# ilur98/DLMC-QUANT

Hardware: AMD Instinct MI355X
Metric: ResNet-50 W8A8 fake-quant fwd images/sec (higher is better)
Workload: dtype i8; 1 GPU; resnet50 W8A8 per-channel fake-quant forward (FSPTQ forms: W minmax_channel s8, A minmax_tensor u8), BN folded first as in FSPTQuant.py:67, fused int8 MFMA conv/linear, frozen execution plan (epilogue-fused ReLU / shortcut / next-layer codes; block end + next 1x1 as one launch; weight codes quantised once at plan build), 2 HIP streams per GPU, 224x224 relu(N(0,1)) pixels, batch 512 per GPU, scales; global_batch=512, parallelism=dp1 (batch-sharded replicas)

## Files before the change

### dlmc-quant_amd/csrc/conv3x3_i8.hip

```cpp
#include "conv_i8_common.h"

namespace dlmcq {

struct HaloGeom {
  int N, H, W, C, K;
  int Hin, Win;
  int Wp, FS;
  uint32_t MQ;
  int nblk_n;
  int hp;
  FastDiv fsdiv, wpdiv;
};

constexpr int halo_tap(bool s2, int t) { return !s2 ? t : (t == 0 ? 4 : t == 1 ? 3 : t == 2 ? 5 : t == 3 ? 1 : t == 4 ? 7 : t == 5 ? 0 : t == 6 ? 2 : t == 7 ? 6 : 8); }
constexpr int halo_ph(bool s2, int t) { return !s2 ? 0 : (t == 0 ? 0 : t <= 2 ? 1 : t <= 4 ? 2 : 3); }
constexpr int halo_rs(bool s2, int t) { return !s2 ? t / 3 : (halo_tap(true, t) / 3 > 0 ? 1 : 0); }
constexpr int halo_cs(bool s2, int t) { return !s2 ? t % 3 : (halo_tap(true, t) % 3 > 0 ? 1 : 0); }

template <int BN, int TM, int NW, int WC, int HPW, int NHB, int WPE, bool XS, int LAB = 0, bool S2 = false, int HPA = HPW * NW, bool PLAIN = false>
__global__ __launch_bounds__(NW * 64, WPE) void conv3x3_halo_i8_kernel(
    const int8_t* __restrict__ x, const int8_t* __restrict__ w, const float* __restrict__ bias, const int32_t* __restrict__ wsum,
    const float* __restrict__ s_in, const float* __restrict__ zp_in, const float* __restrict__ s_w, HaloGeom g, int shift, ConvEpi ep,
    unsigned long long* __restrict__ trace) {
  constexpr bool STAMP = LAB == 1;
  if (LAB >= 9 && LAB <= 11 && blockIdx.x >= 256 && blockIdx.x < 512) {
    for (int i = 0; i < (LAB == 9 ? 4 : LAB == 10 ? 2 : 8); ++i) __builtin_amdgcn_s_sleep(127);
  }
  if ((LAB == 12 || LAB == 13) && blockIdx.x < 1024) {
    for (int i = 0; i < (int)((blockIdx.x >> 8) & 3u); ++i) {
      if (LAB == 12) __builtin_amdgcn_s_sleep(127);
      else __builtin_amdgcn_s_sleep(63);
    }
  }
  const unsigned long long t_start = STAMP ? __builtin_readcyclecounter() : 0ull;
  constexpr int NT = NW * 64;
  constexpr int NBUF = 3;
  constexpr int SLAB = BN * 64;
  constexpr int WPX = NW / WC;
  constexpr int PW = TM / WPX;
  constexpr int CW = BN / WC;
  constexpr int PB = PW / 32, CB = CW / 32;
  constexpr int HP = HPA;
  constexpr int HALO = HP * 1024;
  constexpr int NBW = SLAB / 1024 / NW;
  constexpr int RING = NBUF * SLAB;
  constexpr int SROW = BN + 16;
  constexpr int STAGE = TM * SROW;
  constexpr int OPER = RING + NHB * HALO;
  constexpr int LDS_BYTES = OPER < STAGE ? STAGE : OPER;
  constexpr int PAR_BYTES = 3 * BN * 4;
  static_assert(PB >= 1 && CB >= 1 && NBW >= 1 && NBW * NW * 1024 == SLAB && HPW <= 8 && BN % 64 == 0 && (S2 ? NHB == 3 : (NHB == 1 || NHB == 2)) && HPA <= HPW * NW, "tile shape");
  __shared__ __attribute__((aligned(1024))) int8_t lds[LDS_BYTES + PAR_BYTES];
  int8_t* const ring = lds;
  int8_t* const halo = lds + RING;
  int8_t* const par = lds + LDS_BYTES;
  const uint32_t nwg = gridDim.x;
  const uint32_t xcd = blockIdx.x & 7u, slot = blockIdx.x >> 3;
  const uint32_t qd = nwg >> 3, rm = nwg & 7u;
  const uint32_t tile = (xcd < rm ? xcd * (qd + 1) : rm * (qd + 1) + (xcd - rm) * qd) + slot;
  const int bn = tile % g.nblk_n, bm = tile / g.nblk_n;
  const uint32_t q0 = (uint32_t)bm * TM;
  const int n0 = bn * BN;

  const int tid = threadIdx.x, wave = __builtin_amdgcn_readfirstlane(tid >> 6), lane = tid & 63, l31 = lane & 31, hsel = lane >> 5;
  const int wc = wave % WC, wp = wave / WC;
  unsigned long long* const wgt = (STAMP && tid == 0) ? trace + 64 * 8 + 6 * (size_t)blockIdx.x : nullptr;
  unsigned long long* const stp = (STAMP && tid == 0 && blockIdx.x == gridDim.x / 2) ? trace : nullptr;
  if (STAMP && wgt) {
    wgt[0] = t_start;
    wgt[4] = __builtin_amdgcn_s_memrealtime();
  }
  int stepno = 0;
  auto stamp = [&](int k) {
    if (STAMP && stp && stepno < 64) stp[stepno * 8 + k] = __builtin_readcyclecounter();
  };

  {
    const void* arrs[3] = {s_w, wsum, bias};
#pragma unroll
    for (int a = 0; a < 3; ++a) {
      if (!arrs[a]) continue;
#pragma unroll
      for (int c = 0; c < BN / 64; ++c) {
        if (((a * (BN / 64) + c) % NW) != wave) continue;
        __builtin_amdgcn_global_load_lds((gptr_t)(static_cast<const int32_t*>(arrs[a]) + n0 + c * 64 + lane),
                                         (lptr_t)(par + (a * BN + c * 64) * 4), 4, 0, 0);
      }
    }
  }
  const float zpf = zp_in ? zp_in[0] : 0.0f;
  const int zpi = (int)__builtin_rintf(zpf);
  const float sin_early = s_in[0];
  const uint32_t xorw = 0x80808080u;
  const int8_t* const padline = g_pad_table.b + ((zpi & 0xff) << 6);

  const int lrow = lane >> 2, pslot = lane & 3;
  const int8_t* hsrc[HPW];
  int hinc[HPW];
  int hpc[HPW];
#pragma unroll
  for (int i = 0; i < HPW; ++i) {
    int pc = i * NW + wave;
    pc = pc < g.hp ? pc : g.hp - 1;
    hpc[i] = pc;
    const int p = pc * 16 + lrow;
    const uint32_t f = q0 + (uint32_t)p;
    const uint32_t n = fdiv(f, g.fsdiv);
    const uint32_t rem = f - n * (uint32_t)g.FS;
    const uint32_t fy = fdiv(rem, g.wpdiv);
    const uint32_t fx = rem - fy * (uint32_t)g.Wp;
    const bool in = n < (uint32_t)g.N && fy >= 1u && fx >= 1u;
    const int seg = pslot ^ ((p >> 2) & 3);
    if constexpr (S2) {
      hsrc[i] = in ? x + ((int64_t)((n * (uint32_t)g.Hin + 2u * (fy - 1u)) * (uint32_t)g.Win + 2u * (fx - 1u))) * g.C + seg * 16 : padline;
      hinc[i] = in ? -1 : 0;
    } else {
      hsrc[i] = in ? x + ((int64_t)((n * (uint32_t)g.H + fy - 1u) * (uint32_t)g.W + fx - 1u)) * g.C + seg * 16 : padline;
      hinc[i] = in ? 64 : 0;
    }
  }
  auto issue_halo = [&](auto i_c, int buf) {
    constexpr int i = decltype(i_c)::value;
    if (LAB != 3) __builtin_amdgcn_global_load_lds((gptr_t)hsrc[i], (lptr_t)(halo + buf * HALO + hpc[i] * 1024), 16, 0, 0);
    hsrc[i] += hinc[i];
  };
  const int ph_row = g.Win * g.C, ph_col = g.C;
  auto issue_tile = [&](int ph, int c, int buf) {
    const int off = (ph >> 1) * ph_row + (ph & 1) * ph_col + c * 64;
    static_for<HPW>([&](auto i_c) {
      constexpr int i = decltype(i_c)::value;
      if (LAB != 3) __builtin_amdgcn_global_load_lds((gptr_t)(hsrc[i] + (off & hinc[i])), (lptr_t)(halo + buf * HALO + hpc[i] * 1024), 16, 0, 0);
    });
  };

  const int8_t* wsrc[NBW];
#pragma unroll
  for (int j = 0; j < NBW; ++j) {
    const int drow = (j * NW + wave) * 16 + lrow, d = drow & 31;
    const int k = n0 + (drow & ~31) + 16 * ((d >> 2) & 1) + 4 * (d >> 3) + (d & 3);
    wsrc[j] = w + (int64_t)k * (9 * g.C) + halo_tap(S2, 0) * g.C + (pslot ^ ((drow >> 2) & 3)) * 16;
  }
  const int nchunks = g.C >> 6;
  auto issue_w = [&](auto slot_c, auto u_c) {
    constexpr int SL = decltype(slot_c)::value, u = decltype(u_c)::value;
    constexpr int dtap = u == 8 ? halo_tap(S2, 0) - halo_tap(S2, 8) : halo_tap(S2, (u + 1) % 9) - halo_tap(S2, u);
    const int inc = dtap * g.C + (u == 8 ? 64 : 0);
#pragma unroll
    for (int j = 0; j < NBW; ++j) {
      if (LAB != 2) __builtin_amdgcn_global_load_lds((gptr_t)wsrc[j], (lptr_t)(ring + SL * SLAB + (j * NW + wave) * 1024), 16, 0, 0);
      wsrc[j] += inc;
    }
  };

  int woff[2];
  {
    const int d = wc * CW + l31;
    woff[0] = d * 64 + ((hsel ^ ((d >> 2) & 3)) << 4);
    woff[1] = woff[0] ^ 32;
  }
  const int pbase = wp * PW + l31;
  const int tap_r1 = g.Wp, tap_r2 = 2 * g.Wp;

  i32x16 acc[CB][PB];
#pragma unroll
  for (int jc = 0; jc < CB; ++jc)
#pragma unroll
    for (int jp = 0; jp < PB; ++jp)
#pragma unroll
      for (int i = 0; i < 16; ++i) acc[jc][jp][i] = 0;

  i32x4 wfA[CB], pfA[PB], wfB[CB], pfB[PB];
  auto read_frags = [&](auto u_c, auto t_c, auto ks_c, const int8_t* hbuf, i32x4 (&wf)[CB], i32x4 (&pf)[PB]) {
    constexpr int U = decltype(u_c)::value, t = decltype(t_c)::value, ks = decltype(ks_c)::value;
    const int p0 = pbase + (halo_rs(S2, t) == 0 ? 0 : (halo_rs(S2, t) == 1 ? tap_r1 : tap_r2)) + halo_cs(S2, t);
    const int pa = (p0 * 64 + ((hsel ^ ((p0 >> 2) & 3)) << 4)) ^ (ks << 5);
    const int8_t* const sb = ring + U * SLAB;
#pragma unroll
    for (int jc = 0; jc < CB; ++jc) wf[jc] = *reinterpret_cast<const i32x4*>(sb + woff[ks] + jc * 2048);
#pragma unroll
    for (int jp = 0; jp < PB; ++jp) pf[jp] = *reinterpret_cast<const i32x4*>(hbuf + pa + jp * 2048);
  };
  auto multiply = [&](const i32x4 (&wf)[CB], i32x4 (&pf)[PB]) {
    if (XS && LAB != 6) {
#pragma unroll
      for (int jp = 0; jp < PB; ++jp)
        pf[jp] = i32x4{(int)(pf[jp].x ^ xorw), (int)(pf[jp].y ^ xorw), (int)(pf[jp].z ^ xorw), (int)(pf[jp].w ^ xorw)};
    }
#pragma unroll
    for (int jc = 0; jc < CB; ++jc)
#pragma unroll
      for (int jp = 0; jp < PB; ++jp) {
        if (LAB == 4) asm volatile("" ::"v"(wf[jc]), "v"(pf[jp]));
        else acc[jc][jp] = __builtin_amdgcn_mfma_i32_32x32x32_i8(wf[jc], pf[jp], acc[jc][jp], 0, 0, 0);
      }
  };
  constexpr int nbw = (LAB == 2 ? 0 : NBW);

  if constexpr (S2) {
    issue_tile(0, 0, 0);
    issue_tile(1, 0, 1);
    issue_tile(2, 0, 2);
  } else {
    static_for<HPW>([&](auto i) { issue_halo(i, 0); });
  }
  issue_w(std::integral_constant<int, 0>{}, std::integral_constant<int, 0>{});
  issue_w(std::integral_constant<int, 1>{}, std::integral_constant<int, 1>{});
  issue_w(std::integral_constant<int, 2>{}, std::integral_constant<int, 2>{});
  if (STAMP && wgt) wgt[1] = __builtin_readcyclecounter();
  asm volatile("s_waitcnt vmcnt(%0)\n\ts_barrier" ::"n"(2 * nbw) : "memory");
  if (tid < BN) {
    float* pf = reinterpret_cast<float*>(par) + tid;
    int* pi = reinterpret_cast<int*>(par) + BN + tid;
    *pf = sin_early * *pf;
    *pi = (shift - zpi) * *pi;
  }
  read_frags(std::integral_constant<int, 0>{}, std::integral_constant<int, 0>{}, std::integral_constant<int, 0>{}, halo, wfA, pfA);

  for (int c = 0; c < (NHB == 1 ? 1 : nchunks); ++c) {
    const bool more = NHB != 1 && c + 1 < nchunks;
    const int b0 = S2 ? c % 3 : (NHB == 2 ? (c & 1) : 0);
    auto tile_of = [&](int ph, bool next_chunk) -> const int8_t* {
      if constexpr (S2) {
        int b = b0 + ph + (next_chunk ? 1 : 0);
        b = b >= 6 ? b - 6 : (b >= 3 ? b - 3 : b);
        return halo + b * HALO;
      } else {
        return halo + (NHB == 2 ? ((next_chunk ? c + 1 : c) & 1) * HALO : 0);
      }
    };
    static_for<9>([&](auto t_c) {
      constexpr int t = decltype(t_c)::value;
      constexpr int U = t % NBUF;
      stamp(0);
      read_frags(std::integral_constant<int, U>{}, t_c, std::integral_constant<int, 1>{}, tile_of(halo_ph(S2, t), false), wfB, pfB);
      multiply(wfA, pfA);
      stamp(1);
      if (t < 8 || more) {
        constexpr int hw = (LAB == 3 ? 0 : (S2 ? HPW : 1));
        if constexpr (S2) {
          if (t >= 7 && !more) asm volatile("s_waitcnt vmcnt(0) lgkmcnt(0)\n\ts_barrier" ::: "memory");
          else if (t == 1 || (t == 0 && c > 0) || ((t == 3 || t == 5) && more))
            asm volatile("s_waitcnt vmcnt(%0) lgkmcnt(0)\n\ts_barrier" ::"n"(nbw + hw) : "memory");
          else asm volatile("s_waitcnt vmcnt(%0) lgkmcnt(0)\n\ts_barrier" ::"n"(nbw) : "memory");
        } else {
          constexpr bool HPREV = t >= 1 && t <= HPW && t <= 7;
          if (t >= 7 && !more) asm volatile("s_waitcnt vmcnt(0) lgkmcnt(0)\n\ts_barrier" ::: "memory");
          else if (HPREV && more) asm volatile("s_waitcnt vmcnt(%0) lgkmcnt(0)\n\ts_barrier" ::"n"(nbw + hw) : "memory");
          else asm volatile("s_waitcnt vmcnt(%0) lgkmcnt(0)\n\ts_barrier" ::"n"(nbw) : "memory");
        }
        stamp(2);
        read_frags(std::integral_constant<int, (U + 1) % NBUF>{}, std::integral_constant<int, (t + 1) % 9>{}, std::integral_constant<int, 0>{},
                   tile_of(halo_ph(S2, (t + 1) % 9), t == 8), wfA, pfA);
        if constexpr (S2) {
          if constexpr (t == 0) issue_tile(3, c, b0);
          if constexpr (t == 2 || t == 4 || t == 8) {
            if (more) issue_tile(t == 2 ? 0 : (t == 4 ? 1 : 2), c + 1, (b0 + (t == 2 ? 1 : (t == 4 ? 2 : 0))) % 3);
          }
        } else if constexpr (t < HPW && NHB == 2) {
          if (more) issue_halo(t_c, (c + 1) & 1);
        }
        if (t < 6 || more) issue_w(std::integral_constant<int, U>{}, std::integral_constant<int, (t + 3) % 9>{});
        stamp(3);
      }
      multiply(wfB, pfB);
      if (STAMP) {
        asm volatile("s_nop 0" ::"v"(acc[0][0][0]), "v"(acc[CB - 1][PB - 1][15]));
        stamp(4);
        ++stepno;
      }
    });
  }
  if (STAMP && wgt) wgt[2] = __builtin_readcyclecounter();

  asm volatile("s_barrier" ::: "memory");
  const EpiQuant eq(ep, ep.relu != 0);
  int8_t* const stg = lds;
  auto row_addr = [&](int rr, bool& ok) -> uint8_t* {
    const uint32_t q = q0 + (uint32_t)rr;
    const uint32_t n = fdiv(q, g.fsdiv);
    const uint32_t rem = q - n * (uint32_t)g.FS;
    const uint32_t yy = fdiv(rem, g.wpdiv);
    const uint32_t xx = rem - yy * (uint32_t)g.Wp;
    ok = q < g.MQ && yy < (uint32_t)g.H && xx < (uint32_t)g.W;
    return ep.codes + ((int64_t)((n * (uint32_t)g.H + yy) * (uint32_t)g.W + xx)) * g.K + n0;
  };
#pragma unroll
  for (int jp = 0; jp < PB; ++jp) {
    bool ok8 = false;
    uint8_t* dst8 = nullptr;
    if (LAB == 8) dst8 = row_addr(wp * PW + jp * 32 + l31, ok8);
#pragma unroll
    for (int jc = 0; jc < CB; ++jc) {
      const int cb = wc * CW + jc * 32 + hsel * 16;
      f32x4 y[4];
#pragma unroll
      for (int q = 0; q < 4; ++q) {
        const f32x4 mu = *reinterpret_cast<const f32x4*>(par + (cb + 4 * q) * 4);
        const i32x4 co = *reinterpret_cast<const i32x4*>(par + (BN + cb + 4 * q) * 4);
        const f32x4 bs = bias ? *reinterpret_cast<const f32x4*>(par + (2 * BN + cb + 4 * q) * 4) : f32x4{0.0f, 0.0f, 0.0f, 0.0f};
        if constexpr (PLAIN) {
          const f32x2 ya = pk_fma(f32x2{(float)(acc[jc][jp][4 * q] + co.x), (float)(acc[jc][jp][4 * q + 1] + co.y)}, f32x2{mu.x, mu.y}, f32x2{bs.x, bs.y});
          const f32x2 yb = pk_fma(f32x2{(float)(acc[jc][jp][4 * q + 2] + co.z), (float)(acc[jc][jp][4 * q + 3] + co.w)}, f32x2{mu.z, mu.w}, f32x2{bs.z, bs.w});
          y[q] = f32x4{ya.x, ya.y, yb.x, yb.y};
        } else {
          y[q] = f32x4{dequant1(acc[jc][jp][4 * q] + co.x, mu.x, bs.x), dequant1(acc[jc][jp][4 * q + 1] + co.y, mu.y, bs.y),
                       dequant1(acc[jc][jp][4 * q + 2] + co.z, mu.z, bs.z), dequant1(acc[jc][jp][4 * q + 3] + co.w, mu.w, bs.w)};
        }
      }
      uint32_t wq[4];
      bool uq[4];
      if (LAB == 7) {
#pragma unroll
        for (int q = 0; q < 4; ++q) wq[q] = __builtin_bit_cast(uint32_t, y[q].x + y[q].y + y[q].z + y[q].w);
      } else if constexpr (PLAIN) eq.code4n_plain(y, wq);
      else eq.code4n(y, wq, uq);
      const i32x4 c16 = i32x4{(int)wq[0], (int)wq[1], (int)wq[2], (int)wq[3]};
      if (LAB == 8) {
        if (ok8) __builtin_nontemporal_store(c16, reinterpret_cast<i32x4*>(dst8 + cb));
      } else *reinterpret_cast<i32x4*>(stg + (wp * PW + jp * 32 + l31) * SROW + cb) = c16;
    }
  }
  if (LAB != 8) {
    constexpr int LPR = BN / 16;
    if constexpr (WC == 1) {
      asm volatile("s_waitcnt lgkmcnt(0)" ::: "memory");
      constexpr int RPP = 64 / LPR;
      const int srow = lane / LPR, sseg = lane % LPR;
#pragma unroll
      for (int it = 0; it < PW / RPP; ++it) {
        const int rr = wp * PW + it * RPP + srow;
        bool ok;
        uint8_t* const dst = row_addr(rr, ok);
        const i32x4 c16 = *reinterpret_cast<const i32x4*>(stg + rr * SROW + sseg * 16);
        if (ok) __builtin_nontemporal_store(c16, reinterpret_cast<i32x4*>(dst + sseg * 16));
      }
    } else {
      __syncthreads();
      constexpr int RPP = NT / LPR;
      const int srow = tid / LPR, sseg = tid % LPR;
#pragma unroll
      for (int it = 0; it < TM / RPP; ++it) {
        const int rr = it * RPP + srow;
        bool ok;
        uint8_t* const dst = row_addr(rr, ok);
        const i32x4 c16 = *reinterpret_cast<const i32x4*>(stg + rr * SROW + sseg * 16);
        if (ok) __builtin_nontemporal_store(c16, reinterpret_cast<i32x4*>(dst + sseg * 16));
      }
    }
  }
  if (STAMP && wgt) {
    asm volatile("s_waitcnt vmcnt(0)" ::: "memory");
    wgt[3] = __builtin_readcyclecounter();
    wgt[5] = __builtin_amdgcn_s_memrealtime();
  }
}

bool conv3x3_halo_applies(int64_t N, int64_t H, int64_t W, int64_t C, int64_t K, int64_t R, int64_t S, int32_t stride, int32_t pad,
                          int32_t dilation, const ConvEpi& ep, const float* out, bool dual) {
  if (R != 3 || S != 3 || (stride != 1 && stride != 2) || pad != 1 || dilation != 1 || dual || out || ep.residual || ep.w_off || !ep.codes)
    return false;
  if (C % 64 != 0 || K % 64 != 0 || !aligned16(ep.codes)) return false;
  if (ep.relu == DLMCQ_ACT_RELU6) return false;
  if (stride == 2 && ((H | W) & 1)) return false;
  const int64_t P = H / stride, Q = W / stride;
  if (stride == 2 && Q + 1 > 62) return false;
  if (stride == 2 && C == 64 && K != 64) return false;
  if (Q + 1 > 120 || N * (P + 1) * (Q + 1) + 1024 >= (1ll << 31) || N * H * W * C >= (1ll << 31)) return false;
  return true;
}

int conv3x3_halo_launch(const int8_t* x, const int8_t* w, const float* bias, const int32_t* wsum, const float* in_scale,
                        const float* in_zero_point, const float* w_scale, int64_t N, int64_t H, int64_t W, int64_t C, int64_t K,
                        int32_t stride, int shift, const ConvEpi& ep, hipStream_t st, int lab, void* lab_trace) {
  constexpr int TM = 256;
  const int bn = K % 128 == 0 ? 128 : 64;
  const bool s2 = stride == 2;
  const bool plain = epi_plain(ep);
  HaloGeom g;
  g.N = (int)N; g.Hin = (int)H; g.Win = (int)W; g.H = (int)(H / stride); g.W = (int)(W / stride); g.C = (int)C; g.K = (int)K;
  g.Wp = g.W + 1;
  g.FS = (g.H + 1) * (g.W + 1);
  g.MQ = (uint32_t)(N * g.FS);
  g.nblk_n = (int)(K / bn);
  g.hp = (TM + (s2 ? 1 : 2) * g.Wp + 2 + 15) / 16;
  g.fsdiv = make_fastdiv((uint32_t)g.FS);
  g.wpdiv = make_fastdiv((uint32_t)g.Wp);
  const int64_t nblk_m = ((int64_t)g.MQ + TM - 1) / TM;
  const int64_t nwg = nblk_m * g.nblk_n;
  if (nwg >= (1ll << 31)) return DLMCQ_ERANGE;
  unsigned long long* const trace = static_cast<unsigned long long*>(lab_trace);
#define DLMCQ_HALO_ARGS(NW) dim3((uint32_t)nwg), dim3(NW * 64), 0, st, x, w, bias, wsum, in_scale, in_zero_point, w_scale, g, shift, ep, trace
#ifdef DLMCQ_LAB
  if (lab) {
    const int v = lab % 100;
    if (s2 || g.hp > 24 || (v == 1 && !trace)) return DLMCQ_EINVAL;
    if (lab >= 100) {
      if (bn != 128) return DLMCQ_EINVAL;
      switch (v) {
#define DLMCQ_HALO_LAB(V) case V: hipLaunchKernelGGL((conv3x3_halo_i8_kernel<128, TM, 8, 2, 3, 2, 4, true, V>), DLMCQ_HALO_ARGS(8)); break
        DLMCQ_HALO_LAB(0); DLMCQ_HALO_LAB(1); DLMCQ_HALO_LAB(4);
#undef DLMCQ_HALO_LAB
        default: return DLMCQ_EINVAL;
      }
    } else if (bn == 128) {
      switch (v) {
#define DLMCQ_HALO_LAB(V) case V: hipLaunchKernelGGL((conv3x3_halo_i8_kernel<128, TM, 4, 1, 6, 2, 2, true, V>), DLMCQ_HALO_ARGS(4)); break
        DLMCQ_HALO_LAB(1); DLMCQ_HALO_LAB(2); DLMCQ_HALO_LAB(3); DLMCQ_HALO_LAB(4); DLMCQ_HALO_LAB(6); DLMCQ_HALO_LAB(7); DLMCQ_HALO_LAB(8);
        DLMCQ_HALO_LAB(9); DLMCQ_HALO_LAB(10); DLMCQ_HALO_LAB(11);
#undef DLMCQ_HALO_LAB
        default: return DLMCQ_EINVAL;
      }
    } else {
      if (C != 64) return DLMCQ_EINVAL;
      switch (v) {
#define DLMCQ_HALO_LAB(V) case V: hipLaunchKernelGGL((conv3x3_halo_i8_kernel<64, TM, 4, 1, 6, 1, 4, true, V>), DLMCQ_HALO_ARGS(4)); break
        DLMCQ_HALO_LAB(1); DLMCQ_HALO_LAB(2); DLMCQ_HALO_LAB(3); DLMCQ_HALO_LAB(4); DLMCQ_HALO_LAB(6); DLMCQ_HALO_LAB(7); DLMCQ_HALO_LAB(8);
        DLMCQ_HALO_LAB(12); DLMCQ_HALO_LAB(13);
#undef DLMCQ_HALO_LAB
        default: return DLMCQ_EINVAL;
      }
    }
    return launch_status();
  }
#else
  if (lab) return DLMCQ_EINVAL;
#endif
#define DLMCQ_HALO_GO(NW, ...)                                                                            \
  do {                                                                                                   \
    if (shift) hipLaunchKernelGGL((conv3x3_halo_i8_kernel<__VA_ARGS__>), DLMCQ_HALO_ARGS(NW));           \
    else hipLaunchKernelGGL((conv3x3_halo_i8_kernel<__VA_ARGS__>), DLMCQ_HALO_ARGS(NW));                 \
  } while (0)
  if (s2) {
    if (g.hp > 20) return DLMCQ_EINVAL;
    const bool big = g.hp > 18;
#define DLMCQ_HALO_S2(BN_, HPA_, WPE_)                                                                                                         \
  do {                                                                                                                                        \
    if (shift && plain) hipLaunchKernelGGL((conv3x3_halo_i8_kernel<BN_, TM, 4, 1, 5, 3, WPE_, true, 0, true, HPA_, true>), DLMCQ_HALO_ARGS(4));  \
    else if (shift) hipLaunchKernelGGL((conv3x3_halo_i8_kernel<BN_, TM, 4, 1, 5, 3, WPE_, true, 0, true, HPA_>), DLMCQ_HALO_ARGS(4));            \
    else if (plain) hipLaunchKernelGGL((conv3x3_halo_i8_kernel<BN_, TM, 4, 1, 5, 3, WPE_, false, 0, true, HPA_, true>), DLMCQ_HALO_ARGS(4));     \
    else hipLaunchKernelGGL((conv3x3_halo_i8_kernel<BN_, TM, 4, 1, 5, 3, WPE_, false, 0, true, HPA_>), DLMCQ_HALO_ARGS(4));                      \
  } while (0)
    if (bn == 128) {
      if (!big) DLMCQ_HALO_S2(128, 18, 2);
      else DLMCQ_HALO_S2(128, 20, 1);
    } else {
      if (!big) DLMCQ_HALO_S2(64, 18, 2);
      else DLMCQ_HALO_S2(64, 20, 2);
    }
#undef DLMCQ_HALO_S2
    return launch_status();
  }
  if (g.hp > 32) return DLMCQ_EINVAL;
  const bool wide = g.hp > 24;
#undef DLMCQ_HALO_GO
#define DLMCQ_HALO_GO(BN_, HPW_, NHB_, WPE_)                                                                                                              \
  do {                                                                                                                                                   \
    if (shift && plain) hipLaunchKernelGGL((conv3x3_halo_i8_kernel<BN_, TM, 4, 1, HPW_, NHB_, WPE_, true, 0, false, 4 * HPW_, true>), DLMCQ_HALO_ARGS(4));  \
    else if (shift) hipLaunchKernelGGL((conv3x3_halo_i8_kernel<BN_, TM, 4, 1, HPW_, NHB_, WPE_, true>), DLMCQ_HALO_ARGS(4));                                \
    else if (plain) hipLaunchKernelGGL((conv3x3_halo_i8_kernel<BN_, TM, 4, 1, HPW_, NHB_, WPE_, false, 0, false, 4 * HPW_, true>), DLMCQ_HALO_ARGS(4));     \
    else hipLaunchKernelGGL((conv3x3_halo_i8_kernel<BN_, TM, 4, 1, HPW_, NHB_, WPE_, false>), DLMCQ_HALO_ARGS(4));                                          \
  } while (0)
  if (bn == 128) {
    if (!wide) DLMCQ_HALO_GO(128, 6, 2, 2);
    else DLMCQ_HALO_GO(128, 8, 2, 1);
  } else if (C == 64) {
    if (!wide) DLMCQ_HALO_GO(64, 6, 1, 4);
    else DLMCQ_HALO_GO(64, 8, 1, 3);
  } else {
    if (!wide) DLMCQ_HALO_GO(64, 6, 2, 2);
    else DLMCQ_HALO_GO(64, 8, 2, 2);
  }
#undef DLMCQ_HALO_GO
#undef DLMCQ_HALO_ARGS
  return launch_status();
}

}
```

Before: 92800 images/s.

## Add dense output-row tiling for 3x3 halo conv to skip padded frame rows

Adds a DENSE variant of the stride-1 3x3 halo conv kernel. Its M tiles cover only real output pixels (N*H*W) rather than the padded (H+1)*(W+1) frame, so the padding rows and columns of each frame are no longer computed and then discarded. Each pixel row gets its own halo offset, and a host-side router picks dense or frame layout and a TM of 128 or 256 from halo span, K divisibility and CU count. The cost is per-fragment address math with one LDS read per jp, extra launch variants, and an env-var override.

```diff
diff --git a/dlmc-quant_amd/csrc/conv3x3_i8.hip b/dlmc-quant_amd/csrc/conv3x3_i8.hip
--- a/dlmc-quant_amd/csrc/conv3x3_i8.hip
+++ b/dlmc-quant_amd/csrc/conv3x3_i8.hip
@@ -1,3 +1,6 @@
+#include <cstdlib>
+#include <cstring>
+
 #include "conv_i8_common.h"
 
 namespace dlmcq {
@@ -10,14 +13,23 @@
   int nblk_n;
   int hp;
   FastDiv fsdiv, wpdiv;
+  uint32_t MP;
+  int HW;
+  FastDiv hwdiv, wdiv;
 };
+
+__device__ __forceinline__ uint32_t halo_frame_of(const HaloGeom& g, uint32_t m) {
+  const uint32_t n = fdiv(m, g.hwdiv);
+  const uint32_t rem = m - n * (uint32_t)g.HW;
+  return n * (uint32_t)g.FS + rem + fdiv(rem, g.wdiv);
+}
 
 constexpr int halo_tap(bool s2, int t) { return !s2 ? t : (t == 0 ? 4 : t == 1 ? 3 : t == 2 ? 5 : t == 3 ? 1 : t == 4 ? 7 : t == 5 ? 0 : t == 6 ? 2 : t == 7 ? 6 : 8); }
 constexpr int halo_ph(bool s2, int t) { return !s2 ? 0 : (t == 0 ? 0 : t <= 2 ? 1 : t <= 4 ? 2 : 3); }
 constexpr int halo_rs(bool s2, int t) { return !s2 ? t / 3 : (halo_tap(true, t) / 3 > 0 ? 1 : 0); }
 constexpr int halo_cs(bool s2, int t) { return !s2 ? t % 3 : (halo_tap(true, t) % 3 > 0 ? 1 : 0); }
 
-template <int BN, int TM, int NW, int WC, int HPW, int NHB, int WPE, bool XS, int LAB = 0, bool S2 = false, int HPA = HPW * NW, bool PLAIN = false>
+template <int BN, int TM, int NW, int WC, int HPW, int NHB, int WPE, bool XS, int LAB = 0, bool S2 = false, int HPA = HPW * NW, bool PLAIN = false, bool DENSE = false>
 __global__ __launch_bounds__(NW * 64, WPE) void conv3x3_halo_i8_kernel(
     const int8_t* __restrict__ x, const int8_t* __restrict__ w, const float* __restrict__ bias, const int32_t* __restrict__ wsum,
     const float* __restrict__ s_in, const float* __restrict__ zp_in, const float* __restrict__ s_w, HaloGeom g, int shift, ConvEpi ep,
@@ -49,7 +61,7 @@
   constexpr int OPER = RING + NHB * HALO;
   constexpr int LDS_BYTES = OPER < STAGE ? STAGE : OPER;
   constexpr int PAR_BYTES = 3 * BN * 4;
-  static_assert(PB >= 1 && CB >= 1 && NBW >= 1 && NBW * NW * 1024 == SLAB && HPW <= 8 && BN % 64 == 0 && (S2 ? NHB == 3 : (NHB == 1 || NHB == 2)) && HPA <= HPW * NW, "tile shape");
+  static_assert(PB >= 1 && CB >= 1 && NBW >= 1 && NBW * NW * 1024 == SLAB && HPW <= 8 && BN % 64 == 0 && (S2 ? NHB == 3 : (NHB == 1 || NHB == 2)) && HPA <= HPW * NW && !(DENSE && S2), "tile shape");
   __shared__ __attribute__((aligned(1024))) int8_t lds[LDS_BYTES + PAR_BYTES];
   int8_t* const ring = lds;
   int8_t* const halo = lds + RING;
@@ -59,7 +71,8 @@
   const uint32_t qd = nwg >> 3, rm = nwg & 7u;
   const uint32_t tile = (xcd < rm ? xcd * (qd + 1) : rm * (qd + 1) + (xcd - rm) * qd) + slot;
   const int bn = tile % g.nblk_n, bm = tile / g.nblk_n;
-  const uint32_t q0 = (uint32_t)bm * TM;
+  const uint32_t m0 = (uint32_t)bm * TM;
+  const uint32_t q0 = DENSE ? halo_frame_of(g, m0) : m0;
   const int n0 = bn * BN;
 
   const int tid = threadIdx.x, wave = __builtin_amdgcn_readfirstlane(tid >> 6), lane = tid & 63, l31 = lane & 31, hsel = lane >> 5;
@@ -160,6 +173,14 @@
   }
   const int pbase = wp * PW + l31;
   const int tap_r1 = g.Wp, tap_r2 = 2 * g.Wp;
+  int ppos[PB];
+  if constexpr (DENSE) {
+#pragma unroll
+    for (int jp = 0; jp < PB; ++jp) {
+      const uint32_t m = m0 + (uint32_t)(wp * PW + jp * 32 + l31);
+      ppos[jp] = (int)(halo_frame_of(g, m < g.MP ? m : g.MP - 1u) - q0);
+    }
+  }
 
   i32x16 acc[CB][PB];
 #pragma unroll
@@ -172,13 +193,22 @@
   i32x4 wfA[CB], pfA[PB], wfB[CB], pfB[PB];
   auto read_frags = [&](auto u_c, auto t_c, auto ks_c, const int8_t* hbuf, i32x4 (&wf)[CB], i32x4 (&pf)[PB]) {
     constexpr int U = decltype(u_c)::value, t = decltype(t_c)::value, ks = decltype(ks_c)::value;
-    const int p0 = pbase + (halo_rs(S2, t) == 0 ? 0 : (halo_rs(S2, t) == 1 ? tap_r1 : tap_r2)) + halo_cs(S2, t);
-    const int pa = (p0 * 64 + ((hsel ^ ((p0 >> 2) & 3)) << 4)) ^ (ks << 5);
+    const int sh = (halo_rs(S2, t) == 0 ? 0 : (halo_rs(S2, t) == 1 ? tap_r1 : tap_r2)) + halo_cs(S2, t);
     const int8_t* const sb = ring + U * SLAB;
 #pragma unroll
     for (int jc = 0; jc < CB; ++jc) wf[jc] = *reinterpret_cast<const i32x4*>(sb + woff[ks] + jc * 2048);
-#pragma unroll
-    for (int jp = 0; jp < PB; ++jp) pf[jp] = *reinterpret_cast<const i32x4*>(hbuf + pa + jp * 2048);
+    if constexpr (DENSE) {
+#pragma unroll
+      for (int jp = 0; jp < PB; ++jp) {
+        const int p0 = ppos[jp] + sh;
+        pf[jp] = *reinterpret_cast<const i32x4*>(hbuf + ((p0 * 64 + ((hsel ^ ((p0 >> 2) & 3)) << 4)) ^ (ks << 5)));
+      }
+    } else {
+      const int p0 = pbase + sh;
+      const int pa = (p0 * 64 + ((hsel ^ ((p0 >> 2) & 3)) << 4)) ^ (ks << 5);
+#pragma unroll
+      for (int jp = 0; jp < PB; ++jp) pf[jp] = *reinterpret_cast<const i32x4*>(hbuf + pa + jp * 2048);
+    }
   };
   auto multiply = [&](const i32x4 (&wf)[CB], i32x4 (&pf)[PB]) {
     if (XS && LAB != 6) {
@@ -276,13 +306,19 @@
   const EpiQuant eq(ep, ep.relu != 0);
   int8_t* const stg = lds;
   auto row_addr = [&](int rr, bool& ok) -> uint8_t* {
-    const uint32_t q = q0 + (uint32_t)rr;
-    const uint32_t n = fdiv(q, g.fsdiv);
-    const uint32_t rem = q - n * (uint32_t)g.FS;
-    const uint32_t yy = fdiv(rem, g.wpdiv);
-    const uint32_t xx = rem - yy * (uint32_t)g.Wp;
-    ok = q < g.MQ && yy < (uint32_t)g.H && xx < (uint32_t)g.W;
-    return ep.codes + ((int64_t)((n * (uint32_t)g.H + yy) * (uint32_t)g.W + xx)) * g.K + n0;
+    if constexpr (DENSE) {
+      const uint32_t m = m0 + (uint32_t)rr;
+      ok = m < g.MP;
+      return ep.codes + (int64_t)m * g.K + n0;
+    } else {
+      const uint32_t q = q0 + (uint32_t)rr;
+      const uint32_t n = fdiv(q, g.fsdiv);
+      const uint32_t rem = q - n * (uint32_t)g.FS;
+      const uint32_t yy = fdiv(rem, g.wpdiv);
+      const uint32_t xx = rem - yy * (uint32_t)g.Wp;
+      ok = q < g.MQ && yy < (uint32_t)g.H && xx < (uint32_t)g.W;
+      return ep.codes + ((int64_t)((n * (uint32_t)g.H + yy) * (uint32_t)g.W + xx)) * g.K + n0;
+    }
   };
 #pragma unroll
   for (int jp = 0; jp < PB; ++jp) {
@@ -367,6 +403,81 @@
   if (stride == 2 && C == 64 && K != 64) return false;
   if (Q + 1 > 120 || N * (P + 1) * (Q + 1) + 1024 >= (1ll << 31) || N * H * W * C >= (1ll << 31)) return false;
   return true;
+}
+
+static int halo_dense_pieces(int64_t N, int H, int W, int TM, int cap) {
+  const int64_t HW = (int64_t)H * W, M = N * HW, Wp = W + 1, FS = (int64_t)(H + 1) * Wp;
+  const int64_t rows = (M < TM ? M : TM) - 1;
+  if (rows + rows / W + 2 * Wp + 3 > (int64_t)cap * 16) return cap + 1;
+  struct Memo { int64_t n; int h, w, tm, cap, pieces; };
+  thread_local Memo memo[16] = {};
+  thread_local int next = 0;
+  for (const Memo& e : memo)
+    if (e.n == N && e.h == H && e.w == W && e.tm == TM && e.cap == cap) return e.pieces;
+  auto frame_of = [&](int64_t m) { const int64_t n = m / HW, rem = m - n * HW; return n * FS + rem + rem / W; };
+  int64_t a = TM, b = HW;
+  while (b) { const int64_t t = a % b; a = b; b = t; }
+  const int64_t ntile = (M + TM - 1) / TM, period = HW / a;
+  int64_t span = 0;
+  for (int64_t t = 0; t < (ntile < period ? ntile : period) && span <= (int64_t)cap * 16; ++t) {
+    const int64_t first = t * TM, last = first + TM - 1 < M ? first + TM - 1 : M - 1;
+    const int64_t sp = frame_of(last) - frame_of(first) + 2 * Wp + 3;
+    span = sp > span ? sp : span;
+  }
+  const int pieces = span > (int64_t)cap * 16 ? cap + 1 : (int)((span + 15) / 16);
+  memo[next] = Memo{N, H, W, TM, cap, pieces};
+  next = (next + 1) & 15;
+  return pieces;
+}
+
+enum { HALO_PIN_FRAME = 1, HALO_PIN_DENSE = 2, HALO_PIN_256 = 4, HALO_PIN_128 = 8 };
+static int halo_pins() {
+  const char* const e = std::getenv("DLMCQ_HALO_FORM");
+  if (!e || !*e) return 0;
+  return (std::strstr(e, "frame") ? HALO_PIN_FRAME : 0) | (std::strstr(e, "dense") ? HALO_PIN_DENSE : 0) |
+         (std::strstr(e, "tm256") ? HALO_PIN_256 : 0) | (std::strstr(e, "tm128") ? HALO_PIN_128 : 0);
+}
+
+struct HaloRoute {
+  bool dense;
+  int tm, hp;
+  int64_t nblk_m;
+};
+
+static bool halo_route(int64_t N, int H, int W, int64_t K, bool s2, HaloRoute& r) {
+  const int Wp = W + 1, pins = halo_pins();
+  const int64_t MQ = N * (int64_t)(H + 1) * Wp, MP = N * (int64_t)H * W;
+  const bool bn128 = K % 128 == 0;
+  auto frame_hp = [&](int tm) { return (tm + (s2 ? 1 : 2) * Wp + 2 + 15) / 16; };
+  auto form = [&](int tm, HaloRoute& o) -> bool {
+    const int cap = tm == 256 ? 24 : 12;
+    const int dp = s2 ? cap + 1 : halo_dense_pieces(N, H, W, tm, cap);
+    const bool dense_ok = dp <= cap, frame_ok = tm == 256 || frame_hp(tm) <= cap;
+    bool dense = dense_ok && bn128;
+    if (pins & HALO_PIN_DENSE) dense = true;
+    if (pins & HALO_PIN_FRAME) dense = false;
+    if (dense ? !dense_ok : !frame_ok) return false;
+    o.dense = dense;
+    o.tm = tm;
+    o.hp = dense ? dp : frame_hp(tm);
+    o.nblk_m = ((dense ? MP : MQ) + tm - 1) / tm;
+    return true;
+  };
+  const bool can128 = !s2 && bn128;
+  if (pins & HALO_PIN_128) return can128 && form(128, r);
+  if (!form(256, r)) return false;
+  if ((pins & HALO_PIN_256) || !can128) return true;
+  const int64_t nwg = r.nblk_m * (K / 128), cus = device_cus();
+  HaloRoute r128;
+  if (nwg < cus && form(128, r128) && (r128.dense || 2 * nwg < cus)) r = r128;
+  return true;
+}
+
+extern "C" __attribute__((visibility("default"))) int64_t dlmcq_x_conv3x3_halo_route(int64_t N, int64_t H, int64_t W, int64_t K, int32_t stride) {
+  HaloRoute r;
+  if (stride != 1 && stride != 2) return DLMCQ_EINVAL;
+  if (!halo_route(N, (int)(H / stride), (int)(W / stride), K, stride == 2, r)) return DLMCQ_EINVAL;
+  return (r.dense ? 1 : 0) | (r.tm == 128 ? 2 : 0) | (r.nblk_m << 8);
 }
 
 int conv3x3_halo_launch(const int8_t* x, const int8_t* w, const float* bias, const int32_t* wsum, const float* in_scale,
@@ -382,11 +493,20 @@
   g.FS = (g.H + 1) * (g.W + 1);
   g.MQ = (uint32_t)(N * g.FS);
   g.nblk_n = (int)(K / bn);
-  g.hp = (TM + (s2 ? 1 : 2) * g.Wp + 2 + 15) / 16;
   g.fsdiv = make_fastdiv((uint32_t)g.FS);
   g.wpdiv = make_fastdiv((uint32_t)g.Wp);
-  const int64_t nblk_m = ((int64_t)g.MQ + TM - 1) / TM;
-  const int64_t nwg = nblk_m * g.nblk_n;
+  g.HW = g.H * g.W;
+  g.MP = (uint32_t)(N * g.HW);
+  g.hwdiv = make_fastdiv((uint32_t)g.HW);
+  g.wdiv = make_fastdiv((uint32_t)g.W);
+  HaloRoute route;
+#ifdef DLMCQ_LAB
+  if (lab) route = HaloRoute{false, TM, (TM + 2 * g.Wp + 2 + 15) / 16, ((int64_t)g.MQ + TM - 1) / TM};
+  else
+#endif
+  if (!halo_route(N, g.H, g.W, K, s2, route)) return DLMCQ_EINVAL;
+  g.hp = route.hp;
+  const int64_t nwg = route.nblk_m * g.nblk_n;
   if (nwg >= (1ll << 31)) return DLMCQ_ERANGE;
   unsigned long long* const trace = static_cast<unsigned long long*>(lab_trace);
 #define DLMCQ_HALO_ARGS(NW) dim3((uint32_t)nwg), dim3(NW * 64), 0, st, x, w, bias, wsum, in_scale, in_zero_point, w_scale, g, shift, ep, trace
@@ -453,23 +573,34 @@
   if (g.hp > 32) return DLMCQ_EINVAL;
   const bool wide = g.hp > 24;
 #undef DLMCQ_HALO_GO
-#define DLMCQ_HALO_GO(BN_, HPW_, NHB_, WPE_)                                                                                                              \
-  do {                                                                                                                                                   \
-    if (shift && plain) hipLaunchKernelGGL((conv3x3_halo_i8_kernel<BN_, TM, 4, 1, HPW_, NHB_, WPE_, true, 0, false, 4 * HPW_, true>), DLMCQ_HALO_ARGS(4));  \
-    else if (shift) hipLaunchKernelGGL((conv3x3_halo_i8_kernel<BN_, TM, 4, 1, HPW_, NHB_, WPE_, true>), DLMCQ_HALO_ARGS(4));                                \
-    else if (plain) hipLaunchKernelGGL((conv3x3_halo_i8_kernel<BN_, TM, 4, 1, HPW_, NHB_, WPE_, false, 0, false, 4 * HPW_, true>), DLMCQ_HALO_ARGS(4));     \
-    else hipLaunchKernelGGL((conv3x3_halo_i8_kernel<BN_, TM, 4, 1, HPW_, NHB_, WPE_, false>), DLMCQ_HALO_ARGS(4));                                          \
+#define DLMCQ_HALO_GO4(BN_, TM_, HPW_, NHB_, WPE_, DENSE_)                                                                                                     \
+  do {                                                                                                                                                        \
+    if (shift && plain) hipLaunchKernelGGL((conv3x3_halo_i8_kernel<BN_, TM_, 4, 1, HPW_, NHB_, WPE_, true, 0, false, 4 * HPW_, true, DENSE_>), DLMCQ_HALO_ARGS(4));  \
+    else if (shift) hipLaunchKernelGGL((conv3x3_halo_i8_kernel<BN_, TM_, 4, 1, HPW_, NHB_, WPE_, true, 0, false, 4 * HPW_, false, DENSE_>), DLMCQ_HALO_ARGS(4));      \
+    else if (plain) hipLaunchKernelGGL((conv3x3_halo_i8_kernel<BN_, TM_, 4, 1, HPW_, NHB_, WPE_, false, 0, false, 4 * HPW_, true, DENSE_>), DLMCQ_HALO_ARGS(4));      \
+    else hipLaunchKernelGGL((conv3x3_halo_i8_kernel<BN_, TM_, 4, 1, HPW_, NHB_, WPE_, false, 0, false, 4 * HPW_, false, DENSE_>), DLMCQ_HALO_ARGS(4));                \
   } while (0)
-  if (bn == 128) {
-    if (!wide) DLMCQ_HALO_GO(128, 6, 2, 2);
+#define DLMCQ_HALO_GO(BN_, HPW_, NHB_, WPE_) DLMCQ_HALO_GO4(BN_, TM, HPW_, NHB_, WPE_, false)
+#define DLMCQ_HALO_GOD(BN_, HPW_, NHB_, WPE_)                        \
+  do {                                                               \
+    if (route.dense) DLMCQ_HALO_GO4(BN_, TM, HPW_, NHB_, WPE_, true); \
+    else DLMCQ_HALO_GO4(BN_, TM, HPW_, NHB_, WPE_, false);            \
+  } while (0)
+  if (route.tm == 128) {
+    if (route.dense) DLMCQ_HALO_GO4(128, 128, 3, 2, 3, true);
+    else DLMCQ_HALO_GO4(128, 128, 3, 2, 3, false);
+  } else if (bn == 128) {
+    if (!wide) DLMCQ_HALO_GOD(128, 6, 2, 2);
     else DLMCQ_HALO_GO(128, 8, 2, 1);
   } else if (C == 64) {
-    if (!wide) DLMCQ_HALO_GO(64, 6, 1, 4);
+    if (!wide) DLMCQ_HALO_GOD(64, 6, 1, 4);
     else DLMCQ_HALO_GO(64, 8, 1, 3);
   } else {
-    if (!wide) DLMCQ_HALO_GO(64, 6, 2, 2);
+    if (!wide) DLMCQ_HALO_GOD(64, 6, 2, 2);
     else DLMCQ_HALO_GO(64, 8, 2, 2);
   }
+#undef DLMCQ_HALO_GOD
+#undef DLMCQ_HALO_GO4
 #undef DLMCQ_HALO_GO
 #undef DLMCQ_HALO_ARGS
   return launch_status();
```

After: 94240 images/s (median of 6 runs). 1.02x the previous value.
